# Sharath-girish/Shacira

Hardware: AMD Instinct MI355X
Metric: hash-grid samples/sec fwd+bwd (16 lvl, F=2) (higher is better)
Workload: dtype f32

## Files before the change

shacira_amd/csrc/bwd_bin_front.h:

```cpp
#pragma once

#include "bwd_bin_types.h"

namespace shacira {

template <typename T, int F, bool GMAX>
__global__ __launch_bounds__(256) void transpose_grad_kernel(const T *__restrict__ go, float *__restrict__ gT,
                                                             int64_t N, int64_t NP, int L, int lb, int le,
                                                             uint32_t *__restrict__ gmax) {
    __shared__ uint32_t s_max[SHACIRA_MAX_LODS];
    if (GMAX && threadIdx.x < SHACIRA_MAX_LODS) s_max[threadIdx.x] = 0;
    struct alignas(sizeof(T) * F) PieceIn { T v[F]; };
    struct alignas(sizeof(float) * F) PieceOut { float v[F]; };
    extern __shared__ __align__(16) unsigned char s_raw_g[];
    PieceOut *s_tile = reinterpret_cast<PieceOut *>(s_raw_g);
    const int pitch = L + 1;
    const int64_t s0 = (int64_t)blockIdx.x * 256;
    const int ns = (int)((N - s0 < 256) ? (N - s0) : 256);
    const PieceIn *in = reinterpret_cast<const PieceIn *>(go) + s0 * L;
    const int total = ns * L;
    for (int e = threadIdx.x; e < total; e += 256) {
        const int sm = e / L, l = e - sm * L;
        const PieceIn p = in[e];
        PieceOut q;
// ... 173 lines not shown
            v += r512;
            if (v >= VPR) { v -= VPR; ++sm; }
        }
        for (int e = (int)threadIdx.x + kFrontThreads * UL; e < total; e += kFrontThreads) {
            park1(__builtin_nontemporal_load(src_of(e, sm, v)), sm, v);
            sm += q512;
            v += r512;
            if (v >= VPR) { v -= VPR; ++sm; }
        }
        lds_barrier();
        if constexpr (COUNT) {
            uint32_t *row = cnt + (size_t)(tile0 + r) * plan.total_buckets;
            const bool close = plan.pad > 1u && ((uint32_t)((tile0 + r + 1) % (int64_t)cps) == 0u || tile0 + r + 1 == tiles);
#pragma unroll
            for (int j = 0; j < HE; ++j) {
                const int hc = hcol_of(j);
                if (hc >= 0) {
                    const uint32_t h = s_hist[threadIdx.x + j * kFrontThreads];
                    s_hist[threadIdx.x + j * kFrontThreads] = 0;
                    row[hc] = h;
                    hacc[j] += h;
                    hsum[j] += h;
                    if (close) {
                        hsum[j] += (0u - hacc[j]) & (plan.pad - 1u);
                        hacc[j] = 0;
                    }
                }
            }
        }
        const int work = (le - lb) << nvec_log2;
        for (int idx = threadIdx.x; idx < work; idx += kFrontThreads) {
            const int l = lb + (idx >> nvec_log2), smo = (idx & ((1 << nvec_log2) - 1)) << M_LOG2;
            uint32_t m = 0;
            if (smo < ns) {
                const f32x4 val = *reinterpret_cast<const f32x4 *>(&s_tile[l * pitch + smo]);
                float *dst = gT + ((int64_t)l * NP + s0 + smo) * F;
                if (smo + M <= ns) {
                    if constexpr (sizeof(T) == 4) *reinterpret_cast<f32x4 *>(dst) = val;
                    else __builtin_nontemporal_store(val, reinterpret_cast<f32x4 *>(dst));
                    if constexpr (GMAX) {
#pragma unroll
                        for (int j = 0; j < 4; ++j) {
                            const uint32_t b = __float_as_uint(fabsf(val[j]));
                            m = b > m ? b : m;
                        }
                    }
                } else {
#pragma unroll
                    for (int j = 0; j < F; ++j) {
                        dst[j] = val[j];
                        if constexpr (GMAX) {
                            const uint32_t b = __float_as_uint(fabsf(val[j]));
                            m = b > m ? b : m;
                        }
                    }
                }
            }
            if constexpr (GMAX) {
#pragma unroll
                for (int off = 32; off > 0; off >>= 1) {
                    const uint32_t o = __shfl_xor(m, off, 64);
                    m = o > m ? o : m;
                }
                if ((threadIdx.x & 63) == 0 && m) atomicMax(&s_max[l], m);
            }
        }
        lds_barrier();
    }
    __syncthreads();
    if constexpr (COUNT) {
        uint32_t *mine = totals + (size_t)(blockIdx.x % kTotalShards) * kMaxBuckets;
#pragma unroll
        for (int j = 0; j < HE; ++j) {
            const int hc = hcol_of(j);
            if (hc >= 0 && hsum[j]) atomicAdd(&mine[hc], hsum[j]);
        }
    }
    if constexpr (GMAX) {
        if ((int)threadIdx.x >= lb && (int)threadIdx.x < le && s_max[threadIdx.x])
            atomicMax(&gmax[threadIdx.x], s_max[threadIdx.x]);
    }
}

__global__ __launch_bounds__(1024) void bin_scan_buckets_kernel(const uint32_t *__restrict__ totals,
                                                                uint64_t *__restrict__ base,
                                                                uint32_t *__restrict__ unit_first,
                                                                UnitDesc *__restrict__ unit_desc, uint32_t nb,
                                                                BinPlan plan,
                                                                uint32_t *__restrict__ work_counter,
                                                                unsigned long long *__restrict__ cursor,
                                                                const uint32_t *__restrict__ gmax) {
    __shared__ uint64_t s_items[kMaxBuckets + 2];
    __shared__ uint32_t s_units[kMaxBuckets + 2];
    __shared__ uint64_t s_wave_items[16];
    __shared__ uint32_t s_wave_units[16];
    const uint32_t t = threadIdx.x, lane = t & 63, wave = t >> 6;
    if (t == 0) work_counter[0] = 0;
    uint64_t c[2];
    uint32_t u[2], lv_of[2], ck[2];
#pragma unroll
    for (int k = 0; k < 2; ++k) {
        const uint32_t b = 2 * t + k;
        c[k] = 0u;
        if (b < nb)
            for (int sh = 0; sh < kTotalShards; ++sh) c[k] += totals[(size_t)sh * kMaxBuckets + b];
        uint32_t lvl = plan.blevel[0];
#pragma unroll
        for (uint32_t q = 1; q < SHACIRA_MAX_LODS; ++q)
            if (q < plan.nbl && plan.bstart[q] <= b) lvl = plan.blevel[q];
        lv_of[k] = lvl;
        ck[k] = plan.chunk;
        u[k] = (c[k] >> 32) ? (uint32_t)((c[k] + ck[k] - 1) / ck[k]) : (c[k] ? ((uint32_t)c[k] - 1u) / ck[k] + 1u : 0u);
    }
    uint64_t ci = c[0] + c[1];
    uint32_t ui = u[0] + u[1];
#pragma unroll
    for (int off = 1; off < 64; off <<= 1) {
        const uint64_t nc = __shfl_up(ci, off, 64);
        const uint32_t nu = __shfl_up(ui, off, 64);
        if (lane >= (uint32_t)off) { ci += nc; ui += nu; }
    }
    if (lane == 63) { s_wave_items[wave] = ci; s_wave_units[wave] = ui; }
    __syncthreads();
    uint64_t wc = 0;
    uint32_t wu = 0;
    for (uint32_t w = 0; w < wave; ++w) { wc += s_wave_items[w]; wu += s_wave_units[w]; }
    const uint64_t ex_items = wc + ci - (c[0] + c[1]);
    const uint32_t ex_units = wu + ui - (u[0] + u[1]);
    s_items[2 * t] = ex_items;
    s_items[2 * t + 1] = ex_items + c[0];
    s_units[2 * t] = ex_units;
    s_units[2 * t + 1] = ex_units + u[0];
    if (t == 1023) {
        s_items[kMaxBuckets] = ex_items + c[0] + c[1];
        s_units[kMaxBuckets] = ex_units + u[0] + u[1];
    }
    __syncthreads();
    for (uint32_t b = t; b <= nb; b += 1024) {
        base[b] = s_items[b];
        cursor[b] = s_items[b];
        unit_first[b] = s_units[b];
    }
#pragma unroll
    for (int k = 0; k < 2; ++k) {
        const uint32_t b = 2 * t + k;
        if (b < nb) {
            const uint32_t lvl = lv_of[k];
            const uint32_t gm = (gmax != nullptr && u[k] > 0) ? gmax[lvl] : 0u;
            for (uint32_t q = 0; q < u[k]; ++q) {
                UnitDesc d;
                d.begin = s_items[b] + (uint64_t)q * ck[k];
                const uint64_t bucket_end = s_items[b] + c[k];
                d.end = (d.begin + ck[k] < bucket_end) ? (d.begin + ck[k]) : bucket_end;
                d.bucket = b;
                d.level = lvl;
                d.single = u[k] == 1 ? 1u : 0u;
                d.gmax_bits = gm;
                unit_desc[s_units[b] + q] = d;
            }
        }
    }
}

template <int DIM>
__global__ __launch_bounds__(kBinThreads) void bin_count_levels_kernel(LevelTable lt, BinPlan plan,
                                                                       const float *__restrict__ coords,
                                                                       uint32_t *__restrict__ totals,
                                                                       uint32_t *__restrict__ cnt, int64_t sample0,
                                                                       int64_t N) {
    __shared__ uint32_t s_hist[SHACIRA_MAX_LODS][kMaxLevelBuckets];
    constexpr int kTileD = TileOf<DIM>::value;
    constexpr int SPT = kTileD / kBinThreads;
    const uint32_t tile = blockIdx.x;
    for (uint32_t e = threadIdx.x; e < plan.nbl * kMaxLevelBuckets; e += kBinThreads) (&s_hist[0][0])[e] = 0;
    double t[SPT][DIM];
    bool live[SPT];
#pragma unroll
    for (int u = 0; u < SPT; ++u) {
        const int64_t i = sample0 + (int64_t)tile * kTileD + threadIdx.x + u * kBinThreads;
        live[u] = i < N;
        load_unit_coords<DIM>(coords, i, N, t[u]);
    }
    __syncthreads();
#pragma unroll 1
    for (uint32_t bi = blockIdx.y; bi < plan.nbl; bi += gridDim.y) {
        const uint32_t lvl = plan.blevel[bi];
        const BinLevel bl = plan.lv[lvl];
        const int32_t res = lt.res[lvl];
        const float hi = lt.hi[lvl];
        const bool dense = lt.dense[lvl] != 0;
#pragma unroll
        for (int u = 0; u < SPT; ++u) {
            if (!live[u]) continue;
            if (bl.compact) {
                if constexpr (DIM == 3) {
                    atomicAdd(&s_hist[bi][axis_pos(t[u][2], res, hi) / bl.slab], 2u);
                } else {
                    atomicAdd(&s_hist[bi][compact2d_line(axis_pos(t[u][1], res, hi), (uint32_t)res) / bl.slab], 1u);
                }
                continue;
            }
            uint32_t bk[1 << (DIM - 1)];
            bool ok[1 << (DIM - 1)];
            enumerate_buckets<DIM>(t[u], res, hi, dense, lt.mask, bl, bk, ok);
#pragma unroll
            for (int q = 0; q < (1 << (DIM - 1)); ++q)
                if (ok[q]) atomicAdd(&s_hist[bi][bk[q]], 1u);
        }
    }
    __syncthreads();
    for (uint32_t bi = blockIdx.y; bi < plan.nbl; bi += gridDim.y) {
        const BinLevel bl = plan.lv[plan.blevel[bi]];
        for (uint32_t b = threadIdx.x; b < bl.nb; b += kBinThreads)
        {
            const uint32_t c = (s_hist[bi][b] + plan.pad - 1u) & ~(plan.pad - 1u);
            cnt[(size_t)tile * plan.total_buckets + bl.bucket0 + b] = s_hist[bi][b];
            if (c)
                atomicAdd(&totals[(size_t)((blockIdx.x + blockIdx.y) % kTotalShards) * kMaxBuckets + bl.bucket0 + b], c);
        }
    }
}

__global__ __launch_bounds__(256) void zero_unowned_rows_kernel(float *__restrict__ acc,
                                                                const int32_t *__restrict__ first_idx, LevelTable lt,
                                                                BinPlan plan, uint32_t *__restrict__ words,
                                                                uint32_t nwords) {
    if ((int)blockIdx.y == lt.num_lods) {
        for (uint32_t i = blockIdx.x * 256 + threadIdx.x; i < nwords; i += gridDim.x * 256) words[i] = 0u;
        return;
    }
    const int l = blockIdx.y, F = lt.feature_dim;
// ... 35 lines not shown
```

shacira_amd/csrc/bwd_bin_passes.h:

```cpp
#pragma once

#include "bwd_bin_types.h"

namespace shacira {

#ifdef SHACIRA_SCATTER_WAVES
#define SHACIRA_SCATTER_ATTR __attribute__((amdgpu_waves_per_eu(SHACIRA_SCATTER_WAVES)))
#else
#define SHACIRA_SCATTER_ATTR
#endif
template <int DIM, int F, int FMT, bool STREAM = true>
__global__ __launch_bounds__((ScatterThreads<DIM, F, FMT>::value)) SHACIRA_SCATTER_ATTR void bin_scatter_kernel(LevelTable lt, BinPlan plan,
                                                                  const float *__restrict__ coords,
                                                                  const float *__restrict__ gT,
                                                                  unsigned long long *__restrict__ cursor,
                                                                  const uint32_t *__restrict__ cnt, uint32_t cps,
                                                                  uint32_t cnt_rows,
                                                                  typename ItemSel<F, FMT>::type *__restrict__ items,
                                                                  int64_t sample0, int64_t N, int64_t gpitch,
                                                                  float *__restrict__ zero_acc,
                                                                  const int32_t *__restrict__ first_idx,
                                                                  const uint32_t *__restrict__ unit_first,
                                                                  int cstride = DIM) {
    typedef typename ItemSel<F, FMT>::type ItemT;
    constexpr bool H = FMT == 1;
    constexpr bool P12 = FMT == 2;
    static_assert(!P12 || (DIM == 3 && F == 2), "12-byte units: 3-D, F = 2");
    constexpr int NP = 1 << (DIM - 1);
    constexpr int kTileD = TileOf<DIM>::value;
    constexpr int kThreads = ScatterThreads<DIM, F, FMT>::value;
    constexpr int SPT = kTileD / kThreads;
    constexpr int kScatterSplit = ScatterSplit<ItemT>::value;
    constexpr int kStage = kTileD * NP / kScatterSplit;
    static_assert(kStage % 2 == 0, "two-slot items never straddle a window");
    extern __shared__ __align__(16) unsigned char s_raw[];
    ItemT *s_items = reinterpret_cast<ItemT *>(s_raw);
    uint8_t *s_bucket = reinterpret_cast<uint8_t *>(s_items + (kScatterSplit == 1 ? plan.stage_cap : (uint32_t)kStage));
    __shared__ uint32_t s_hist[kMaxLevelBuckets];
    __shared__ uint32_t s_start[kMaxLevelBuckets + 1];
    __shared__ uint64_t s_gbase[kMaxLevelBuckets];

#ifdef SCATTER_LEVEL_FAST
    const uint32_t tile = blockIdx.y, bi = blockIdx.x;
#else
    const uint32_t tile = blockIdx.x, bi = blockIdx.y;
#endif
    const uint32_t lvl = plan.blevel[bi];
    const BinLevel bl = plan.lv[lvl];
    if (threadIdx.x < kMaxLevelBuckets) s_hist[threadIdx.x] = 0;
    __syncthreads();
    const int32_t res = lt.res[lvl];
    const float hi = lt.hi[lvl];
    const bool dense = lt.dense[lvl] != 0;

    PairSlot ps[SPT][NP];
    uint32_t rank[SPT][NP];
    float fx[SPT];
    float g[SPT][F];
    float fyz[SPT][2];
    const bool compact = bl.compact != 0;
    constexpr uint32_t kCompactSlots = (DIM == 3) ? 2u : 1u;
    float craw[SPT][DIM], graw[SPT][F];
#pragma unroll
    for (int u = 0; u < SPT; ++u) {
        int64_t i = sample0 + (int64_t)tile * kTileD + threadIdx.x + u * kThreads;
        i = i < N ? i : N - 1;
#ifdef ABL_NO_LOAD
        i = (i * 2654435761ll) & 1023;
#endif
#pragma unroll
        for (int a = 0; a < DIM; ++a) craw[u][a] = coords[i * cstride + a];
        const float *gp = gT + ((int64_t)lvl * gpitch + i) * F;
        if constexpr (F == 2) {
            const float2 v = *reinterpret_cast<const float2 *>(gp);
            graw[u][0] = v.x; graw[u][1] = v.y;
        } else {
#pragma unroll
            for (int j = 0; j < F; ++j) graw[u][j] = gp[j];
        }
    }
    const bool reserver = threadIdx.x >= 64 && threadIdx.x - 64 < bl.nb;
    unsigned long long run_base = 0ull;
    if (reserver) {
        const uint32_t gb = bl.bucket0 + threadIdx.x - 64;
        const uint32_t *row = cnt + (size_t)tile * cps * plan.total_buckets + gb;
        uint32_t c = 0;
        for (uint32_t k = 0; k < cps && tile * cps + k < cnt_rows; ++k) c += row[(size_t)k * plan.total_buckets];
        c = (c + plan.pad - 1u) & ~(plan.pad - 1u);
#ifdef ABL_NO_CURSOR
        if (c) run_base = cursor[gb] + (unsigned long long)tile * c;
#else
        if (c) run_base = atomicAdd(&cursor[gb], (unsigned long long)c);
#endif
    }
#pragma unroll
    for (int u = 0; u < SPT; ++u) {
        const int k = threadIdx.x + u * kThreads;
        const int64_t i = sample0 + (int64_t)tile * kTileD + k;
        const bool live = i < N;
        double t[DIM];
#pragma unroll
        for (int a = 0; a < DIM; ++a) t[a] = axis_unit(craw[u][a]);
#pragma unroll
        for (int j = 0; j < F; ++j) g[u][j] = graw[u][j];
        if (compact) {
            if constexpr (DIM == 3) {
                int32_t pp[3];
                float ff[3], gg[3];
#pragma unroll
                for (int a = 0; a < 3; ++a) axis_transform(t[a], res, hi, pp[a], ff[a], gg[a]);
                const uint32_t r = (uint32_t)res, b = (uint32_t)pp[2] / bl.slab;
                const uint32_t local = ((uint32_t)pp[2] - b * bl.slab) * r * r + (uint32_t)pp[1] * r + (uint32_t)pp[0];
                fx[u] = ff[0];
                fyz[u][0] = ff[1];
                fyz[u][1] = ff[2];
#pragma unroll
                for (int q = 0; q < NP; ++q) {
                    ps[u][q].bucket = b;
                    ps[u][q].key = 0;
                    ps[u][q].wrest = 0.0f;
                }
                ps[u][0].key = local | (1u << 26);
            } else {
                int32_t pp[2];
                float ff[2], gg[2];
#pragma unroll
                for (int a = 0; a < 2; ++a) axis_transform(t[a], res, hi, pp[a], ff[a], gg[a]);
                const uint32_t r = (uint32_t)res, b = compact2d_line((uint32_t)pp[1], r) / bl.slab;
                const uint32_t local = ((uint32_t)pp[1] - b * bl.slab) * r + (uint32_t)pp[0];
                fx[u] = ff[0];
                fyz[u][0] = ff[1];
                fyz[u][1] = 0.0f;
                ps[u][0].bucket = b;
                ps[u][0].key = local | (1u << 26);
                ps[u][0].wrest = 0.0f;
                ps[u][1].bucket = b;
                ps[u][1].key = 0;
                ps[u][1].wrest = 0.0f;
            }
        } else {
            enumerate_pairs<DIM>(t, res, hi, dense, lt.mask, bl, plan.BR, fx[u], ps[u]);
        }
#pragma unroll
        for (int q = 0; q < NP; ++q) {
            if (!live) ps[u][q].key = 0;
            rank[u][q] = (ps[u][q].key >> 26) ? atomicAdd(&s_hist[ps[u][q].bucket], compact ? kCompactSlots : 1u) : 0u;
        }
    }
    lds_barrier();
    if (threadIdx.x < 64) {
        const uint32_t lane = threadIdx.x;
        const uint32_t pm = plan.pad - 1u;
        const uint32_t c0 = (2 * lane < bl.nb) ? ((s_hist[2 * lane] + pm) & ~pm) : 0u;
        const uint32_t c1 = (2 * lane + 1 < bl.nb) ? ((s_hist[2 * lane + 1] + pm) & ~pm) : 0u;
        uint32_t incl = c0 + c1;
#pragma unroll
        for (int off = 1; off < 64; off <<= 1) {
            const uint32_t nbr = __shfl_up(incl, off, 64);
            if (lane >= (uint32_t)off) incl += nbr;
        }
        const uint32_t excl = incl - (c0 + c1);
        if (2 * lane < bl.nb) s_start[2 * lane] = excl;
        if (2 * lane + 1 < bl.nb) s_start[2 * lane + 1] = excl + c0;
        if (lane == 63) s_start[bl.nb] = incl;
    }
    lds_barrier();
    if (kScatterSplit == 1 && plan.pad > 1u && threadIdx.x < bl.nb) {
        const uint32_t b = threadIdx.x;
        for (uint32_t pos = s_start[b] + s_hist[b]; pos < s_start[b + 1]; ++pos) {
            uint32_t *w = reinterpret_cast<uint32_t *>(&s_items[pos]);
#pragma unroll
            for (int k = 0; k < (int)(sizeof(ItemT) / 4); ++k) w[k] = 0u;
            s_bucket[pos] = (uint8_t)b;
        }
    }
    const uint32_t staged = s_start[bl.nb];
// ... 49 lines not shown
                    } else {
                        s_items[pos] = pack_item12(ps[u][q].key, fx[u], dense, g[u][0] * ps[u][q].wrest, g[u][1] * ps[u][q].wrest);
                        s_bucket[pos] = (uint8_t)ps[u][q].bucket;
                    }
                    continue;
                }
                if constexpr (H && F == 2) {
                    if (compact) {
                        ItemHC c;
                        c.key = ps[u][q].key;
                        c.fx = (uint16_t)(fx[u] * 65536.0f);
                        c.fy = (uint16_t)(fyz[u][0] * 65536.0f);
                        c.fz = (uint16_t)(fyz[u][1] * 65536.0f);
                        c.pad = 0;
                        c.g = __floats2half2_rn(g[u][0], g[u][1]);
                        *reinterpret_cast<ItemHC *>(&s_items[pos]) = c;
                        s_bucket[pos] = (uint8_t)ps[u][q].bucket;
                        s_bucket[pos + 1] = (uint8_t)ps[u][q].bucket;
                    } else {
                        ItemH it;
                        it.key = pack_half_key(ps[u][q].key, fx[u], dense);
                        it.a = __floats2half2_rn(g[u][0] * ps[u][q].wrest, g[u][1] * ps[u][q].wrest);
                        s_items[pos] = it;
                        s_bucket[pos] = (uint8_t)ps[u][q].bucket;
                    }
                    continue;
                }
                if constexpr (!H && !P12) {
                Item<F> it;
                it.key = ps[u][q].key;
                it.fx = fx[u];
                if constexpr (DIM == 2 && !H) {
                    if (compact) {
                        uint32_t w0, w1;
                        pack_compact2d(ps[u][q].key, fx[u], fyz[u][0], w0, w1);
                        it.key = w0;
                        it.fx = __uint_as_float(w1);
#pragma unroll
                        for (int j = 0; j < F; ++j) it.a[j] = g[u][j];
                        *reinterpret_cast<Item<F> *>(&s_items[pos]) = it;
                        s_bucket[pos] = (uint8_t)ps[u][q].bucket;
                        continue;
                    }
                }
                if (compact) {
                    if constexpr (F == 2) {
                        it.a[0] = fyz[u][0];
                        it.a[1] = fyz[u][1];
                        *reinterpret_cast<Item<F> *>(&s_items[pos]) = it;
                        Item<F> it2;
                        it2.key = 0;
                        it2.fx = g[u][0];
                        it2.a[0] = g[u][1];
                        it2.a[1] = 0.0f;
                        *reinterpret_cast<Item<F> *>(&s_items[pos + 1]) = it2;
                        s_bucket[pos] = (uint8_t)ps[u][q].bucket;
                        s_bucket[pos + 1] = (uint8_t)ps[u][q].bucket;
                    } else if constexpr (F == 4) {
                        it.a[0] = fyz[u][0];
                        it.a[1] = fyz[u][1];
                        it.a[2] = g[u][0];
                        it.a[3] = g[u][1];
                        *reinterpret_cast<Item<F> *>(&s_items[pos]) = it;
                        Item<F> it2;
                        it2.key = 0;
                        it2.fx = g[u][2];
                        it2.a[0] = g[u][3];
                        it2.a[1] = 0.0f; it2.a[2] = 0.0f; it2.a[3] = 0.0f;
                        *reinterpret_cast<Item<F> *>(&s_items[pos + 1]) = it2;
                        s_bucket[pos] = (uint8_t)ps[u][q].bucket;
                        s_bucket[pos + 1] = (uint8_t)ps[u][q].bucket;
                    }
                } else {
#pragma unroll
                    for (int j = 0; j < F; ++j) it.a[j] = g[u][j] * ps[u][q].wrest;
                    *reinterpret_cast<Item<F> *>(&s_items[pos]) = it;
                    s_bucket[pos] = (uint8_t)ps[u][q].bucket;
                }
                }
            }
        }
    }
    if (wi == 0) {
        if (reserver) s_gbase[threadIdx.x - 64] = run_base;
        __syncthreads();
    } else {
        lds_barrier();
    }
    const uint32_t in_window = (kScatterSplit == 1 || staged - w0 < (uint32_t)kStage) ? (staged - w0) : (uint32_t)kStage;
#ifndef ABL_NO_STORE
    for (uint32_t pos = threadIdx.x; pos < in_window; pos += kThreads) {
        const uint32_t b = s_bucket[pos];
        store_item_nt<STREAM>(items + s_gbase[b] + (w0 + pos - s_start[b]), s_items[pos]);
    }
#endif
    if (kScatterSplit > 1 && wi + 1u < n_win) lds_barrier();
    }
    if (zero_acc != nullptr && !dense) {
        for (uint32_t b = tile; b < bl.nb; b += plan.num_tiles) {
            const uint32_t gb = bl.bucket0 + b;
            if (unit_first[gb + 1] - unit_first[gb] == 1u) continue;
            const uint32_t row0 = b * bl.rows_pb;
            const uint32_t nrows = (bl.used - row0 < bl.rows_pb) ? (bl.used - row0) : bl.rows_pb;
            float *dst = zero_acc + ((int64_t)first_idx[lvl] + row0) * F;
            for (uint32_t e = threadIdx.x; e < nrows * (uint32_t)F; e += kThreads) dst[e] = 0.0f;
        }
    }
}

#ifdef CONSUME_TRACE
__device__ unsigned long long g_consume_trace[16384 * 8];
__device__ unsigned int g_consume_trace_n;
#define CTRACE(k) do { if (threadIdx.x == 0) ctr[k] = wall_clock64(); } while (0)
#else
#define CTRACE(k) do { } while (0)
#endif
template <int F, bool FX, int FMT, class Hook>
__device__ __forceinline__ void consume_unit(const LevelTable &lt, const BinPlan &plan, const int32_t *__restrict__ first_idx,
                                             const UnitDesc d, const typename ItemSel<F, FMT>::type *__restrict__ items,
                                             float *__restrict__ grad_table, int force_atomic, int headroom, double *s_acc,
                                             Hook &&hook, __half *__restrict__ half_out = nullptr) {
    constexpr bool H = FMT == 1;
    constexpr bool P12 = FMT == 2;
    const uint32_t gb = (uint32_t)__builtin_amdgcn_readfirstlane((int)d.bucket);
    const uint32_t lvl = (uint32_t)__builtin_amdgcn_readfirstlane((int)d.level);
    const BinLevel bl = plan.lv[lvl];
    const uint32_t b = gb - bl.bucket0;
    const uint32_t r1 = (uint32_t)lt.res[lvl];
    const bool two_d = plan.pairs == 2u;
    const uint32_t row0 = bl.compact ? b * bl.slab * (two_d ? r1 : r1 * r1) : b * bl.rows_pb;
    const uint32_t nrows = (bl.used - row0 < bl.rows_pb) ? (bl.used - row0) : bl.rows_pb;

    FxScale fx{1.0, 1.0, false};
    if constexpr (FX) fx = fx_scale_of(d.gmax_bits, headroom);
    unsigned long long *s_fix = reinterpret_cast<unsigned long long *>(s_acc);
#ifdef CONSUME_TRACE
    unsigned long long ctr[8] = {0, 0, 0, 0, 0, 0, 0, 0};
    struct TraceOut {
        unsigned long long *c; UnitDesc dd;
        __device__ ~TraceOut() {
            if (threadIdx.x == 0) {
                c[5] = wall_clock64();
                const unsigned int slot = atomicAdd(&g_consume_trace_n, 1u);
                if (slot < 16384u) {
                    unsigned long long *o = g_consume_trace + (size_t)slot * 8;
                    o[0] = ((unsigned long long)dd.level << 32) | dd.bucket;
                    o[1] = dd.end - dd.begin;
                    for (int k = 0; k < 6; ++k) o[2 + k] = c[k];
                }
            }
        }
    } trace_out{ctr, d};
#endif
    CTRACE(0);
    auto zero_image = [&]() {
        for (uint32_t e = threadIdx.x; e < nrows * F; e += kConsumeThreads) s_acc[e] = 0.0;
        lds_barrier();
    };
    const uint64_t begin = d.begin, end = d.end;
    auto stream = [&](uint64_t first, uint64_t lim, uint64_t stride, auto &&load, auto &&proc) {
        uint64_t p0 = first;
        load(p0);
        CTRACE(1);
        zero_image();
        CTRACE(2);
        proc();
        CTRACE(3);
// ... 663 lines not shown
```

shacira_amd/csrc/hashgrid_bwd_bin.hip:

```cpp
#include <mutex>

#include <cstring>

#include "bwd_bin_types.h"
#include "bwd_bin_front.h"
#include "bwd_bin_passes.h"
#include "bwd_brick.h"
#include <hip/hip_ext.h>

namespace shacira {

static inline size_t align_up(size_t v, size_t a) { return (v + a - 1) / a * a; }

static void make_plan(int dim, int dtype, const LevelTable &lt, int64_t n_batch, BinPlan &plan, int acc_kib,
                      bool one_image_compact, uint32_t skip_mask = 0u, int64_t n_call = 0);
static inline bool half_items(int dtype, const LevelTable &lt);
static inline int item_format(int dim, int dtype, const LevelTable &lt, int64_t n);
static inline size_t item_unit_bytes(int fmt, const LevelTable &lt);
#ifndef SHACIRA_RUN_ALIGN
#define SHACIRA_RUN_ALIGN 64
#endif
#ifndef SHACIRA_PAD_HALF
#define SHACIRA_PAD_HALF 0
#endif
// ... 214 lines not shown
        plan.bnb[q] = q < plan.nbl ? plan.lv[plan.blevel[q]].nb : 0u;
    }
    plan.total_buckets = nbk;
    plan.BR = BR;
    plan.num_tiles = (uint32_t)((n_batch + tile_samples(dim) - 1) / tile_samples(dim));
    plan.pairs = 1u << (dim - 1);
    uint64_t chunk = (uint64_t)n_batch * plan.pairs / 48 + 1024;
    if (chunk < 8192) chunk = 8192;
    if (chunk > (1u << 22)) chunk = 1u << 22;
    plan.pad = 1;
    {
        const int fmt_p = item_format(dim, dtype, lt, n_call);
        const size_t unit = item_unit_bytes(fmt_p, lt);
        const uint32_t tile_units = (uint32_t)tile_samples(dim) * plan.pairs;
        uint32_t maxnb = 0;
        for (uint32_t q = 0; q < plan.nbl; ++q) maxnb = plan.lv[plan.blevel[q]].nb > maxnb ? plan.lv[plan.blevel[q]].nb : maxnb;
        bool windows = false;
#ifdef SHACIRA_SCATTER_SPLIT
        windows = SHACIRA_SCATTER_SPLIT > 1;
#endif
        if (opt().bwd_run_pad != 0 && !windows && plan.nbl > 0 && n_call >= SHACIRA_FX_MIN &&
            ((fmt_p != 1 && (unit == 16 || unit == 12)) || (SHACIRA_PAD_HALF && fmt_p == 1 && (unit == 8 || unit == 16)))) {
            const uint32_t P = unit == 12 ? (uint32_t)(SHACIRA_RUN_ALIGN / 4) : (uint32_t)(SHACIRA_RUN_ALIGN / unit);
            const size_t staged = (size_t)(tile_units + maxnb * (P - 1u)) * (unit + 1);
            if (staged <= (size_t)78 * 1024 || (size_t)tile_units * (unit + 1) > (size_t)78 * 1024) plan.pad = P;
        }
        plan.stage_cap = tile_units + maxnb * (plan.pad - 1u);
    }
    const uint32_t cmask = plan.pad > 2u ? plan.pad - 1u : 1u;
    plan.chunk = (uint32_t)chunk & ~cmask;
    for (uint32_t q = 0; q < plan.nbl; ++q) {
        BinLevel &bl = plan.lv[plan.blevel[q]];
        bl.chunk = plan.chunk;
        CountLevel &c = plan.cl[q];
        c.res = lt.res[plan.blevel[q]];
        c.hi = lt.hi[plan.blevel[q]];
        c.shift = bl.shift;
        c.m_lo = (uint32_t)bl.magicG;
        c.m_hi = (uint32_t)(bl.magicG >> 32);
        c.kind = lt.dense[plan.blevel[q]] ? 2u : 0u;
        if (bl.compact) {
            const uint32_t m = ((1u << 18) + bl.slab - 1u) / bl.slab;
            bool exact = m < (1u << 18) || bl.slab == 1;
            for (uint32_t pz = 0; pz < (uint32_t)c.res && exact; ++pz) exact = ((pz * m) >> 18) == pz / bl.slab;
            c.kind = 1u;
            c.m_lo = exact ? m : 0u;
            c.m_hi = bl.slab;
        }
    }
    plan.chunk_min = plan.chunk;
}

static inline bool half_items(int dtype, const LevelTable &lt) {
    return dtype == SHACIRA_F16 && (lt.feature_dim == 2 || lt.feature_dim == 4);
}
static inline int item_format(int dim, int dtype, const LevelTable &lt, int64_t n) {
    if (half_items(dtype, lt)) return 1;
    if (dim == 3 && lt.feature_dim == 2 && dtype == SHACIRA_F32 && n >= SHACIRA_FX_MIN && opt().bwd_item12 == 1) return 2;
    return 0;
}
static inline size_t item_unit_bytes(int fmt, const LevelTable &lt) {
    if (fmt == 1) return lt.feature_dim == 2 ? 8 : 16;
    if (fmt == 2) return 12;
    return 8 + 4 * (size_t)lt.feature_dim;
}

static int64_t bin_batch_samples(int dim, int dtype, const LevelTable &lt, int64_t n) {
    const size_t item = item_unit_bytes(item_format(dim, dtype, lt, n), lt);
    BinPlan plan;
    make_plan(dim, dtype, lt, kTile, plan, choose_acc_kib(dim, dtype, lt, n), one_image_compact_rule(n));
    const size_t per_sample = (size_t)(plan.nbl ? plan.nbl : 1) * (1u << (dim - 1)) * item;
    int64_t cap = (int64_t)(((size_t)opt().bin_batch_mib << 20) / per_sample);
    cap = cap / tile_samples(dim) * tile_samples(dim);
    if (cap < tile_samples(dim)) cap = tile_samples(dim);
    return n < cap ? n : cap;
}

struct BinWorkspace {
    float *gT;
    unsigned char *items;
    uint32_t *totals;
    uint32_t *gmax;
    uint64_t *base;
    unsigned long long *cursor;
    uint32_t *cnt;
    uint32_t *unit_first;
    UnitDesc *unit_desc;
    uint32_t *work_counter;
    float *acc32;
    size_t bytes;
};

static inline int64_t level_pitch(int64_t n) { return (n + 1) & ~(int64_t)1; }

static bool table_all_direct(int dim, int dtype, const LevelTable &lt, int64_t n) {
    LevelTable full = lt;
    full.level_begin = 0;
    full.level_end = lt.num_lods;
    BinPlan plan;
    make_plan(dim, dtype, full, kTile, plan, choose_acc_kib(dim, dtype, full, n), one_image_compact_rule(n));
    return plan.nbl == 0;
}

static uint64_t slots_per_sample(const BinPlan &plan) {
    uint64_t slots = 0;
    for (uint32_t q = 0; q < plan.nbl; ++q) {
        const BinLevel &bl = plan.lv[plan.blevel[q]];
        slots += bl.compact ? (plan.pairs == 4u ? 2u : 1u) : plan.pairs;
    }
    return slots;
}

static int front_tile(int L, int F, uint32_t nbl, int64_t n, size_t *shmem);

static void brick_levels_of_call(int dim, int dtype, const LevelTable &lt, int64_t n, const SortedBatch *sb, bool zero_table,
                                 bool grad_aligned, BrickPlan &brick, uint32_t &skip_mask) {
    brick.nlev = 0;
    skip_mask = 0u;
    if (dim != 3 || sb == nullptr) return;
    const int L = lt.num_lods, F = lt.feature_dim;
    const bool multi = bin_batch_samples(dim, dtype, lt, n) < n;
    const int kvec0 = (int)(16 / ((dtype == SHACIRA_F32 ? 4 : 2) * F));
    const int bopt = opt().bwd_brick;
    const bool wanted = bopt == 1 || (bopt < 0 && F == 2 && dtype == SHACIRA_F32);
    if (!wanted || multi || lt.stage_flags != 0 || !zero_table || n < SHACIRA_FX_MIN || n * L >= ((int64_t)1 << 31) ||
        table_all_direct(dim, dtype, lt, n) || (L % kvec0) != 0 || !grad_aligned)
        return;
    if (!make_brick_plan(lt, n, *sb, opt().bwd_brick_lo, opt().bwd_brick_hi, opt().bwd_brick_span,
                         (size_t)(opt().bwd_brick_fork == 2 ? 30 : 64) * 1024, brick)) {
        brick.nlev = 0;
        return;
    }
    for (uint32_t q = 0; q < brick.nlev; ++q) skip_mask |= 1u << brick.lv[q].level;
    BinPlan rest;
    make_plan(dim, dtype, lt, n, rest, choose_acc_kib(dim, dtype, lt, n), one_image_compact_rule(n), skip_mask, n);
    size_t sh0 = 0;
    if (rest.nbl == 0 || front_tile(L, F, rest.nbl, n, &sh0) <= 0) {
        skip_mask = 0u;
        brick.nlev = 0;
    }
}

static BinWorkspace carve(int dim, int dtype, const LevelTable &lt, int64_t n, void *ws, uint32_t skip_mask = 0u) {
    BinPlan plan;
    const int64_t nb = bin_batch_samples(dim, dtype, lt, n);
    make_plan(dim, dtype, lt, nb, plan, choose_acc_kib(dim, dtype, lt, n), one_image_compact_rule(n), skip_mask, n);
    const size_t item = item_unit_bytes(item_format(dim, dtype, lt, n), lt);
    size_t off = 0;
    auto take = [&](size_t bytes) { size_t o = off; off = align_up(off + bytes, 256); return o; };
    const bool no_stage = table_all_direct(dim, dtype, lt, n);
    const size_t o_gT = take(no_stage ? 0 : (size_t)level_pitch(n) * lt.num_lods * lt.feature_dim * sizeof(float));
    const size_t o_ctrl = take((size_t)(kTotalShards * kMaxBuckets + SHACIRA_MAX_LODS) * sizeof(uint32_t));
    const uint64_t pad_units = (uint64_t)plan.num_tiles * plan.total_buckets * (plan.pad - 1u);
    const size_t o_items = take(((size_t)nb * slots_per_sample(plan) + (size_t)pad_units) * item);
    const size_t o_base = take((size_t)(kMaxBuckets + 2) * sizeof(uint64_t));
    const size_t o_cur = take((size_t)(kMaxBuckets + 2) * sizeof(uint64_t));
    const size_t o_cnt = take((size_t)(nb / 128 + 8) * plan.total_buckets * sizeof(uint32_t));
    const size_t o_unit = take((size_t)(kMaxBuckets + 2) * sizeof(uint32_t));
    const uint64_t max_items_ws = (uint64_t)nb * plan.nbl * plan.pairs + pad_units;
    const size_t o_ub = take((size_t)(max_items_ws / plan.chunk_min + plan.total_buckets + 2) * sizeof(UnitDesc));
    const size_t o_wc = take(256);
    const size_t o_acc = take(dtype == SHACIRA_F16 ? (size_t)lt.table_rows * lt.feature_dim * sizeof(float) : 0);
    BinWorkspace w{};
    unsigned char *p = static_cast<unsigned char *>(ws);
    if (p) {
        w.gT = reinterpret_cast<float *>(p + o_gT);
        w.items = p + o_items;
        w.totals = reinterpret_cast<uint32_t *>(p + o_ctrl);
        w.gmax = w.totals + (size_t)kTotalShards * kMaxBuckets;
        w.base = reinterpret_cast<uint64_t *>(p + o_base);
        w.cursor = reinterpret_cast<unsigned long long *>(p + o_cur);
        w.cnt = reinterpret_cast<uint32_t *>(p + o_cnt);
        w.unit_first = reinterpret_cast<uint32_t *>(p + o_unit);
        w.unit_desc = reinterpret_cast<UnitDesc *>(p + o_ub);
        w.work_counter = reinterpret_cast<uint32_t *>(p + o_wc);
        w.acc32 = reinterpret_cast<float *>(p + o_acc);
    }
    w.bytes = off;
    return w;
}

static void resolve_call(int dim, int dtype, const LevelTable &lt, int64_t n, const SortedBatch *sb, bool zero_table,
                         bool grad_aligned, BrickPlan &brick, uint32_t &skip_mask) {
    const bool auto12 = opt().bwd_item12 < 0;
    if (auto12) {
        const bool brick_shape = sb != nullptr && dim == 3 && lt.feature_dim == 2 && dtype == SHACIRA_F32 &&
                                 lt.level_begin == 0 && lt.level_end == lt.num_lods && lt.stage_flags == 0 && zero_table &&
                                 opt().bwd_brick != 0;
        options_resolve_item12(brick_shape ? 1 : 0);
    }
    brick_levels_of_call(dim, dtype, lt, n, sb, zero_table, grad_aligned, brick, skip_mask);
    if (auto12 && brick.nlev == 0) options_resolve_item12(0);
}
static inline uint32_t carve_skip(int dtype, uint32_t skip_mask) { return dtype == SHACIRA_F32 ? skip_mask : 0u; }

size_t bin_workspace_bytes(int dim, int dtype, const LevelTable &lt, int64_t n) {
    return carve(dim, dtype, lt, n, nullptr).bytes;
}

size_t bin_workspace_bytes_planned(int dim, int dtype, const LevelTable &lt, int64_t n, bool whole, bool grad_aligned) {
    SortedBatch sb{};
    sample_plan_grid(dim, n, sb);
    BrickPlan brick;
    uint32_t skip_mask = 0;
    resolve_call(dim, dtype, lt, n, &sb, whole, grad_aligned, brick, skip_mask);
    return carve(dim, dtype, lt, n, nullptr, carve_skip(dtype, skip_mask)).bytes;
}

float *bin_acc32(int dim, int dtype, const LevelTable &lt, int64_t n, void *workspace) {
    return carve(dim, dtype, lt, n, workspace).acc32;
}

#define SHACIRA_CHECK_LAUNCH()                 \
    do {                                       \
        hipError_t e_ = hipGetLastError();     \
        if (e_ != hipSuccess) return e_;       \
    } while (0)
#define SHACIRA_CHECK(expr)                    \
    do {                                       \
        hipError_t e_ = (expr);                \
        if (e_ != hipSuccess) return e_;       \
    } while (0)

struct SideStream {
    hipStream_t stream = nullptr;
    hipEvent_t fork = nullptr, join = nullptr, staged = nullptr;
    hipEvent_t bfork = nullptr, bjoin = nullptr;
};
static hipError_t side_stream(SideStream **out) {
    static thread_local SideStream per_device[kMaxDevices];
    int dev = 0;
    SHACIRA_CHECK(hipGetDevice(&dev));
    if (dev < 0 || dev >= kMaxDevices) return hipErrorInvalidDevice;
    SideStream &ss = per_device[dev];
    if (!ss.stream) {
        hipStream_t st;
        hipEvent_t a, b, c, d, e;
        SHACIRA_CHECK(hipStreamCreateWithFlags(&st, hipStreamNonBlocking));
        SHACIRA_CHECK(hipEventCreateWithFlags(&a, hipEventDisableTiming));
        SHACIRA_CHECK(hipEventCreateWithFlags(&b, hipEventDisableTiming));
        SHACIRA_CHECK(hipEventCreateWithFlags(&c, hipEventDisableTiming));
        SHACIRA_CHECK(hipEventCreateWithFlags(&d, hipEventDisableTiming));
        SHACIRA_CHECK(hipEventCreateWithFlags(&e, hipEventDisableTiming));
        ss.fork = a;
        ss.join = b;
        ss.staged = c;
        ss.bfork = d;
        ss.bjoin = e;
        ss.stream = st;
    }
    *out = &ss;
    return hipSuccess;
}

// ... 141 lines not shown
                else if (front_counts) SHACIRA_FRONT(__half, false, true);
                else SHACIRA_FRONT(__half, false, false);
            }
#undef SHACIRA_FRONT
#undef SHACIRA_FRONT_SORTED
        } else {
            const uint32_t blocks = (uint32_t)((n + 255) / 256);
            const size_t shmem = (size_t)256 * (L + 1) * F * sizeof(float);
            if (dtype == SHACIRA_F32 && use_fx)
                hipLaunchKernelGGL((transpose_grad_kernel<float, F, true>), dim3(blocks), dim3(256), shmem, s,
                                   static_cast<const float *>(grad_out), w.gT, n, NP, L, t_lb, t_le, w.gmax);
            else if (dtype == SHACIRA_F32)
                hipLaunchKernelGGL((transpose_grad_kernel<float, F, false>), dim3(blocks), dim3(256), shmem, s,
                                   static_cast<const float *>(grad_out), w.gT, n, NP, L, t_lb, t_le, nullptr);
            else if (use_fx)
                hipLaunchKernelGGL((transpose_grad_kernel<__half, F, true>), dim3(blocks), dim3(256), shmem, s,
                                   static_cast<const __half *>(grad_out), w.gT, n, NP, L, t_lb, t_le, w.gmax);
            else
                hipLaunchKernelGGL((transpose_grad_kernel<__half, F, false>), dim3(blocks), dim3(256), shmem, s,
                                   static_cast<const __half *>(grad_out), w.gT, n, NP, L, t_lb, t_le, nullptr);
        }
        SHACIRA_CHECK_LAUNCH();
    }
    if (fork) {
        SHACIRA_CHECK(hipEventRecord(ss->staged, s));
        SHACIRA_CHECK(hipStreamWaitEvent(ss->stream, ss->staged, 0));
    }
    if (brick_mode == 1) SHACIRA_CHECK(fork_brick());
    if (whole.ngroups > 0) {
        const BinPlan &plan = whole;
        uint32_t bpg = (plan.ngroups > 1 ? 256u : 512u) / plan.ngroups;
        const uint32_t need = (uint32_t)((n + 2047) / 2048);
        if (bpg > need) bpg = need;
        if (bpg < 1) bpg = 1;
        const size_t acc_bytes = (size_t)plan.BR * F * sizeof(double);
        const dim3 grid(bpg, plan.ngroups);
        const int headroom = fx_headroom(((uint64_t)n / bpg + kConsumeThreads) * (1u << DIM));
        const uint32_t *gm = (need_T && use_fx) ? w.gmax : nullptr;
        if (need_T)
            hipLaunchKernelGGL((direct_accumulate_kernel<DIM, F, float, true, true>), grid, dim3(kConsumeThreads),
                               acc_bytes, zs, lt, plan, first_idx, cptr, w.gT, acc, n, NP, gm, headroom, cstride);
        else if (dtype == SHACIRA_F32)
            hipLaunchKernelGGL((direct_accumulate_kernel<DIM, F, float, false, true>), grid, dim3(kConsumeThreads),
                               acc_bytes, zs, lt, plan, first_idx, coords, static_cast<const float *>(grad_out), acc, n,
                               NP, gm, headroom);
        else
            hipLaunchKernelGGL((direct_accumulate_kernel<DIM, F, __half, false, true>), grid, dim3(kConsumeThreads),
                               acc_bytes, zs, lt, plan, first_idx, coords, static_cast<const __half *>(grad_out), acc, n,
                               NP, gm, headroom);
        SHACIRA_CHECK_LAUNCH();
    }
    if (fork) SHACIRA_CHECK(hipEventRecord(ss->join, ss->stream));
    if (whole.nbl == 0) return hipSuccess;
    constexpr int NPAIR = 1 << (DIM - 1);
    const int fmt = item_format(DIM, dtype, lt, n);
    const bool half = fmt == 1;
    auto stage_bytes = [&](const BinPlan &pl) -> size_t {
        const size_t isz = fmt == 2 ? sizeof(Item12) : half ? sizeof(typename ItemSel<F, true>::type) : sizeof(Item<F>);
        const int split = half ? ScatterSplit<typename ItemSel<F, true>::type>::value : ScatterSplit<Item<F>>::value;
        const size_t units = split == 1 ? (size_t)pl.stage_cap : (size_t)TileOf<DIM>::value * NPAIR / split;
        return units * (isz + 1);
    };
#ifdef SCATTER_LEVEL_FAST
#define SCATTER_GRID(pl) dim3((pl).nbl, (pl).num_tiles)
#else
#define SCATTER_GRID(pl) dim3((pl).num_tiles, (pl).nbl)
#endif
    bool first_batch = true;
    for (int64_t s0 = 0; s0 < n; s0 += nb) {
        const int64_t hi = (s0 + nb < n) ? (s0 + nb) : n;
        BinPlan plan;
        make_plan(DIM, dtype, lt, hi - s0, plan, acc_kib, oic, skip_mask, n);
        if (!first_batch) {
            hipLaunchKernelGGL(zero_words_kernel, dim3(32), dim3(256), 0, s, w.totals, (uint32_t)kTotalShards * kMaxBuckets);
            SHACIRA_CHECK_LAUNCH();
        }
        const bool fused_now = front_counts && first_batch;
        if (!fused_now) {
            hipLaunchKernelGGL((bin_count_levels_kernel<DIM>), count_grid(plan), dim3(kBinThreads), 0, s, lt, plan, coords,
                               w.totals, w.cnt, s0, hi);
            SHACIRA_CHECK_LAUNCH();
        }
        first_batch = false;
        hipLaunchKernelGGL(bin_scan_buckets_kernel, dim3(1), dim3(1024), 0, s, w.totals, w.base, w.unit_first, w.unit_desc,
                           plan.total_buckets, plan, w.work_counter, w.cursor, use_fx ? w.gmax : nullptr);
        SHACIRA_CHECK_LAUNCH();
        float *zacc = selective ? acc : nullptr;
        const uint32_t cps = fused_now ? (uint32_t)(TileOf<DIM>::value / ts16) : 1u;
        const uint32_t cnt_rows = fused_now ? (uint32_t)((n + ts16 - 1) / ts16) : plan.num_tiles;
        bool fork_signalled = false;
        if (fmt == 2) {
            if constexpr (DIM == 3 && F == 2) {
                hipStreamCaptureStatus cap = hipStreamCaptureStatusNone;
                if (brick_mode == 2 && opt().bwd_ext_fork != 0 && hipStreamIsCapturing(s, &cap) == hipSuccess &&
                    cap == hipStreamCaptureStatusNone) {
                    hipExtLaunchKernelGGL((bin_scatter_kernel<DIM, F, 2>), SCATTER_GRID(plan),
                                          dim3(ScatterThreads<DIM, F, 2>::value), (uint32_t)stage_bytes(plan), s, nullptr,
                                          bss->bfork, 0u, lt, plan, cptr, (const float *)w.gT, w.cursor, (const uint32_t *)w.cnt, cps, cnt_rows,
                                          reinterpret_cast<Item12 *>(w.items), s0, hi, NP, zacc, first_idx,
                                          (const uint32_t *)w.unit_first, cstride);
                    fork_signalled = true;
                } else {
                    hipLaunchKernelGGL((bin_scatter_kernel<DIM, F, 2>), SCATTER_GRID(plan), dim3(ScatterThreads<DIM, F, 2>::value),
                                       stage_bytes(plan), s, lt, plan, cptr, w.gT, w.cursor, w.cnt, cps, cnt_rows,
                                       reinterpret_cast<Item12 *>(w.items), s0, hi, NP, zacc, first_idx, w.unit_first, cstride);
                }
            }
        } else if (half)
            hipLaunchKernelGGL((bin_scatter_kernel<DIM, F, true>), SCATTER_GRID(plan), dim3(ScatterThreads<DIM, F, 1>::value),
                               stage_bytes(plan), s, lt, plan, cptr, w.gT, w.cursor, w.cnt, cps, cnt_rows,
                               reinterpret_cast<typename ItemSel<F, true>::type *>(w.items), s0, hi, NP, zacc, first_idx,
                               w.unit_first, cstride);
        else if (use_fx)
            hipLaunchKernelGGL((bin_scatter_kernel<DIM, F, false>), SCATTER_GRID(plan), dim3(ScatterThreads<DIM, F, 0>::value),
                               stage_bytes(plan), s, lt, plan, cptr, w.gT, w.cursor, w.cnt, cps, cnt_rows,
                               reinterpret_cast<Item<F> *>(w.items), s0, hi, NP, zacc, first_idx, w.unit_first, cstride);
        else
            hipLaunchKernelGGL((bin_scatter_kernel<DIM, F, false, false>), SCATTER_GRID(plan), dim3(ScatterThreads<DIM, F, 0>::value),
                               stage_bytes(plan), s, lt, plan, cptr, w.gT, w.cursor, w.cnt, cps, cnt_rows,
                               reinterpret_cast<Item<F> *>(w.items), s0, hi, NP, zacc, first_idx, w.unit_first, cstride);
        SHACIRA_CHECK_LAUNCH();
        if (fork) SHACIRA_CHECK(hipStreamWaitEvent(s, ss->join, 0));
        if (brick_mode == 2) {
            if (fork_signalled) {
                SHACIRA_CHECK(hipStreamWaitEvent(bss->stream, bss->bfork, 0));
                SHACIRA_CHECK(launch_brick(bss->stream, bss->bjoin));
            } else {
                SHACIRA_CHECK(fork_brick());
            }
        }
        const uint64_t max_items = (uint64_t)(hi - s0) * plan.nbl * NPAIR +
                                   (uint64_t)plan.num_tiles * plan.total_buckets * (plan.pad - 1u);
        uint32_t grid_units = (uint32_t)(max_items / plan.chunk_min) + plan.total_buckets + 1;
        const size_t acc_bytes = (size_t)plan.BR * F * sizeof(double);
        uint32_t *wc = (opt().bwd_persistent != 0 && n >= SHACIRA_PERSIST_MIN) ? w.work_counter : nullptr;
        if (wc != nullptr && grid_units > 512u) grid_units = 512u;
        const int headroom = use_fx ? fx_headroom((uint64_t)plan.chunk + 1) : -1;
        const int fa = multi ? 1 : 0;
        __half *hout = direct_half ? half_table : nullptr;
        if (fmt == 2) {
            if constexpr (DIM == 3 && F == 2)
                hipLaunchKernelGGL((bin_consume_kernel<F, true, 2>), dim3(grid_units), dim3(kConsumeThreads), acc_bytes, s, lt,
                                   plan, first_idx, w.unit_first, w.unit_desc, reinterpret_cast<const Item12 *>(w.items), acc,
                                   fa, headroom, wc);
        } else if (half && use_fx)
            hipLaunchKernelGGL((bin_consume_kernel<F, true, true>), dim3(grid_units), dim3(kConsumeThreads), acc_bytes, s,
                               lt, plan, first_idx, w.unit_first, w.unit_desc,
                               reinterpret_cast<const typename ItemSel<F, true>::type *>(w.items), acc, fa, headroom, wc, hout);
        else if (half)
            hipLaunchKernelGGL((bin_consume_kernel<F, false, true>), dim3(grid_units), dim3(kConsumeThreads), acc_bytes, s,
                               lt, plan, first_idx, w.unit_first, w.unit_desc,
                               reinterpret_cast<const typename ItemSel<F, true>::type *>(w.items), acc, fa, headroom, wc, hout);
        else if (use_fx)
            hipLaunchKernelGGL((bin_consume_kernel<F, true, false>), dim3(grid_units), dim3(kConsumeThreads), acc_bytes, s, lt,
                               plan, first_idx, w.unit_first, w.unit_desc,
                               reinterpret_cast<const Item<F> *>(w.items), acc, fa, headroom, wc);
        else if (!half)
            hipLaunchKernelGGL((bin_consume_kernel<F, false, false>), dim3(grid_units), dim3(kConsumeThreads), acc_bytes, s, lt,
                               plan, first_idx, w.unit_first, w.unit_desc,
                               reinterpret_cast<const Item<F> *>(w.items), acc, fa, headroom, wc);
        SHACIRA_CHECK_LAUNCH();
    }
    if (brick_mode == 0) SHACIRA_CHECK(launch_brick(s));
    if (brick_mode > 0) SHACIRA_CHECK(hipStreamWaitEvent(s, bss->bjoin, 0));
    if (direct_half) {
        hipLaunchKernelGGL(f32_to_f16_skip_kernel, dim3(128, (uint32_t)L), dim3(256), 0, s, acc, half_table, first_idx, lt,
                           whole, w.unit_first, F);
        SHACIRA_CHECK_LAUNCH();
        if (converted != nullptr) *converted = true;
    }
    return hipSuccess;
}

template <class ItemT> static constexpr size_t stage_max(size_t tile_units) {
    constexpr size_t split = ScatterSplit<ItemT>::value;
    constexpr size_t padu = split != 1 ? 0 : sizeof(ItemT) == 16 ? SHACIRA_RUN_ALIGN / 16 - 1 : sizeof(ItemT) == 12 ? SHACIRA_RUN_ALIGN / 4 - 1
                            : (SHACIRA_PAD_HALF && sizeof(ItemT) == 8) ? SHACIRA_RUN_ALIGN / 8 - 1 : 0;
    return (tile_units / split + (size_t)kMaxLevelBuckets * padu) * (sizeof(ItemT) + 1);
}

hipError_t bin_backward(int dim, int dtype, const LevelTable &lt, const int32_t *first_idx, const float *coords,
                        const void *grad_out, float *acc, void *workspace, int64_t n, hipStream_t s, bool zero_table,
                        void *half_table, bool *converted, const SortedBatch *sb) {
    if (converted != nullptr) *converted = false;
    __half *ht = (dtype == SHACIRA_F16) ? static_cast<__half *>(half_table) : nullptr;
    BrickPlan brick;
    uint32_t skip_mask = 0;
    resolve_call(dim, dtype, lt, n, sb, zero_table, (reinterpret_cast<uintptr_t>(grad_out) & 15u) == 0, brick, skip_mask);
    const BinWorkspace w = carve(dim, dtype, lt, n, workspace, carve_skip(dtype, skip_mask));
    static PerDeviceOnce once;
    const hipError_t attr_err = once.run([]() -> hipError_t {
        hipError_t attr_err = hipSuccess;
        auto set = [&attr_err](const void *fn, size_t bytes) {
            if (bytes <= 64 * 1024 || bytes > 160 * 1024) return;
            hipError_t e = hipFuncSetAttribute(fn, hipFuncAttributeMaxDynamicSharedMemorySize, (int)bytes);
            if (e != hipSuccess) attr_err = e;
        };
#define SHACIRA_T_ATTR(TT, FF)                                                                           \
        set(reinterpret_cast<const void *>(&transpose_grad_kernel<TT, FF, true>), 140 * 1024);          \
        set(reinterpret_cast<const void *>(&transpose_grad_kernel<TT, FF, false>), 140 * 1024);         \
        set(reinterpret_cast<const void *>(&front16_kernel<2, TT, FF, true, true>), 156 * 1024);        \
        set(reinterpret_cast<const void *>(&front16_kernel<2, TT, FF, true, false>), 156 * 1024);       \
// ... 66 lines not shown
```

Baseline: 1.415 billion.

## Replace per-tile atomic cursor reservation with deterministic prefix-scanned run offsets

```diff
diff --git a/shacira_amd/csrc/bwd_bin_front.h b/shacira_amd/csrc/bwd_bin_front.h
--- a/shacira_amd/csrc/bwd_bin_front.h
+++ b/shacira_amd/csrc/bwd_bin_front.h
@@ -279,14 +279,82 @@
     }
 }
 
-__global__ __launch_bounds__(1024) void bin_scan_buckets_kernel(const uint32_t *__restrict__ totals,
-                                                                uint64_t *__restrict__ base,
-                                                                uint32_t *__restrict__ unit_first,
-                                                                UnitDesc *__restrict__ unit_desc, uint32_t nb,
-                                                                BinPlan plan,
-                                                                uint32_t *__restrict__ work_counter,
-                                                                unsigned long long *__restrict__ cursor,
-                                                                const uint32_t *__restrict__ gmax) {
+constexpr int kScanThreads = 1024;
+constexpr int kScanCols = 16;
+constexpr int kScanChunks = kScanThreads / kScanCols;
+constexpr int kScanRows = 32;
+static_assert(kScanChunks == 64, "one wave scans one column's chunk sums");
+__device__ __forceinline__ void scan_run_offsets(uint32_t *__restrict__ cnt, uint32_t group, uint32_t nb, uint32_t pad,
+                                                 uint32_t cps, uint32_t cnt_rows) {
+    __shared__ uint32_t s_chunk[kScanCols][kScanChunks + 1];
+    const uint32_t col = threadIdx.x % kScanCols, chunk = threadIdx.x / kScanCols;
+    const uint32_t lane = threadIdx.x & 63, wave = threadIdx.x >> 6;
+    const uint32_t gb = group * kScanCols + col;
+    const bool live = gb < nb;
+    uint32_t *colp = cnt + (live ? gb : nb - 1u);
+    const uint32_t pm = pad - 1u;
+    uint32_t carry = 0;
+    for (uint32_t row0 = 0; row0 < cnt_rows; row0 += (uint32_t)(kScanChunks * kScanRows)) {
+        const uint32_t r0 = row0 + chunk * (uint32_t)kScanRows;
+        const uint32_t left = r0 < cnt_rows ? cnt_rows - r0 : 0u;
+        const uint32_t nvalid = left < (uint32_t)kScanRows ? left : (uint32_t)kScanRows;
+        const uint32_t *p = colp + (size_t)(nvalid ? r0 : cnt_rows - 1u) * nb;
+        uint32_t v[kScanRows];
+#pragma unroll
+        for (int k = 0; k < kScanRows; ++k) {
+            v[k] = *p;
+            p += ((uint32_t)k + 1u < nvalid) ? nb : 0u;
+        }
+        uint32_t run = 0, acc = 0;
+#pragma unroll
+        for (int k = 0; k < kScanRows; ++k) {
+            const uint32_t h = ((uint32_t)k < nvalid) ? v[k] : 0u;
+            v[k] = run;
+            acc += h;
+            if ((((uint32_t)k + 1u) & (cps - 1u)) == 0u) {
+                run += (acc + pm) & ~pm;
+                acc = 0;
+            }
+        }
+        s_chunk[col][chunk] = run;
+        __syncthreads();
+        {
+            const uint32_t t = s_chunk[wave][lane];
+            uint32_t incl = t;
+#pragma unroll
+            for (int off = 1; off < 64; off <<= 1) {
+                const uint32_t nbr = __shfl_up(incl, off, 64);
+                if (lane >= (uint32_t)off) incl += nbr;
+            }
+            s_chunk[wave][lane] = incl - t;
+            if (lane == 63) s_chunk[wave][kScanChunks] = incl;
+        }
+        __syncthreads();
+        const uint32_t off0 = carry + s_chunk[col][chunk];
+        carry += s_chunk[col][kScanChunks];
+        uint32_t *w = colp + (size_t)r0 * nb;
+#pragma unroll
+        for (int k = 0; k < kScanRows; ++k) {
+            if (((uint32_t)k & (cps - 1u)) == 0u && (uint32_t)k < nvalid && live) *w = off0 + v[k];
+            w += nb;
+        }
+        __syncthreads();
+    }
+}
+
+__global__ __launch_bounds__(kScanThreads) void bin_scan_buckets_kernel(const uint32_t *__restrict__ totals,
+                                                                        uint64_t *__restrict__ base,
+                                                                        uint32_t *__restrict__ unit_first,
+                                                                        UnitDesc *__restrict__ unit_desc, uint32_t nb,
+                                                                        BinPlan plan,
+                                                                        uint32_t *__restrict__ work_counter,
+                                                                        const uint32_t *__restrict__ gmax,
+                                                                        uint32_t *__restrict__ cnt, uint32_t cps,
+                                                                        uint32_t cnt_rows) {
+    if (blockIdx.x != 0) {
+        scan_run_offsets(cnt, blockIdx.x - 1u, nb, plan.pad, cps, cnt_rows);
+        return;
+    }
     __shared__ uint64_t s_items[kMaxBuckets + 2];
     __shared__ uint32_t s_units[kMaxBuckets + 2];
     __shared__ uint64_t s_wave_items[16];
@@ -294,7 +362,7 @@
     const uint32_t t = threadIdx.x, lane = t & 63, wave = t >> 6;
     if (t == 0) work_counter[0] = 0;
     uint64_t c[2];
-    uint32_t u[2], lv_of[2], ck[2];
+    uint32_t u[2], lv_of[2], ck[2], gm_of[2];
 #pragma unroll
     for (int k = 0; k < 2; ++k) {
         const uint32_t b = 2 * t + k;
@@ -306,6 +374,7 @@
         for (uint32_t q = 1; q < SHACIRA_MAX_LODS; ++q)
             if (q < plan.nbl && plan.bstart[q] <= b) lvl = plan.blevel[q];
         lv_of[k] = lvl;
+        gm_of[k] = gmax != nullptr ? gmax[lvl] : 0u;
         ck[k] = plan.chunk;
         u[k] = (c[k] >> 32) ? (uint32_t)((c[k] + ck[k] - 1) / ck[k]) : (c[k] ? ((uint32_t)c[k] - 1u) / ck[k] + 1u : 0u);
     }
@@ -335,7 +404,6 @@
     __syncthreads();
     for (uint32_t b = t; b <= nb; b += 1024) {
         base[b] = s_items[b];
-        cursor[b] = s_items[b];
         unit_first[b] = s_units[b];
     }
 #pragma unroll
@@ -343,7 +411,7 @@
         const uint32_t b = 2 * t + k;
         if (b < nb) {
             const uint32_t lvl = lv_of[k];
-            const uint32_t gm = (gmax != nullptr && u[k] > 0) ? gmax[lvl] : 0u;
+            const uint32_t gm = gm_of[k];
             for (uint32_t q = 0; q < u[k]; ++q) {
                 UnitDesc d;
                 d.begin = s_items[b] + (uint64_t)q * ck[k];
diff --git a/shacira_amd/csrc/bwd_bin_passes.h b/shacira_amd/csrc/bwd_bin_passes.h
--- a/shacira_amd/csrc/bwd_bin_passes.h
+++ b/shacira_amd/csrc/bwd_bin_passes.h
@@ -13,9 +13,8 @@
 __global__ __launch_bounds__((ScatterThreads<DIM, F, FMT>::value)) SHACIRA_SCATTER_ATTR void bin_scatter_kernel(LevelTable lt, BinPlan plan,
                                                                   const float *__restrict__ coords,
                                                                   const float *__restrict__ gT,
-                                                                  unsigned long long *__restrict__ cursor,
-                                                                  const uint32_t *__restrict__ cnt, uint32_t cps,
-                                                                  uint32_t cnt_rows,
+                                                                  const uint64_t *__restrict__ base,
+                                                                  const uint32_t *__restrict__ run_off, uint32_t cps,
                                                                   typename ItemSel<F, FMT>::type *__restrict__ items,
                                                                   int64_t sample0, int64_t N, int64_t gpitch,
                                                                   float *__restrict__ zero_acc,
@@ -79,19 +78,11 @@
             for (int j = 0; j < F; ++j) graw[u][j] = gp[j];
         }
     }
-    const bool reserver = threadIdx.x >= 64 && threadIdx.x - 64 < bl.nb;
-    unsigned long long run_base = 0ull;
-    if (reserver) {
+    const bool placer = threadIdx.x >= 64 && threadIdx.x - 64 < bl.nb;
+    uint64_t run_base = 0ull;
+    if (placer) {
         const uint32_t gb = bl.bucket0 + threadIdx.x - 64;
-        const uint32_t *row = cnt + (size_t)tile * cps * plan.total_buckets + gb;
-        uint32_t c = 0;
-        for (uint32_t k = 0; k < cps && tile * cps + k < cnt_rows; ++k) c += row[(size_t)k * plan.total_buckets];
-        c = (c + plan.pad - 1u) & ~(plan.pad - 1u);
-#ifdef ABL_NO_CURSOR
-        if (c) run_base = cursor[gb] + (unsigned long long)tile * c;
-#else
-        if (c) run_base = atomicAdd(&cursor[gb], (unsigned long long)c);
-#endif
+        run_base = base[gb] + run_off[(size_t)tile * cps * plan.total_buckets + gb];
     }
 #pragma unroll
     for (int u = 0; u < SPT; ++u) {
@@ -307,7 +298,7 @@
         }
     }
     if (wi == 0) {
-        if (reserver) s_gbase[threadIdx.x - 64] = run_base;
+        if (placer) s_gbase[threadIdx.x - 64] = run_base;
         __syncthreads();
     } else {
         lds_barrier();
diff --git a/shacira_amd/csrc/hashgrid_bwd_bin.hip b/shacira_amd/csrc/hashgrid_bwd_bin.hip
--- a/shacira_amd/csrc/hashgrid_bwd_bin.hip
+++ b/shacira_amd/csrc/hashgrid_bwd_bin.hip
@@ -320,7 +320,6 @@
     uint32_t *totals;
     uint32_t *gmax;
     uint64_t *base;
-    unsigned long long *cursor;
     uint32_t *cnt;
     uint32_t *unit_first;
     UnitDesc *unit_desc;
@@ -392,7 +391,6 @@
     const uint64_t pad_units = (uint64_t)plan.num_tiles * plan.total_buckets * (plan.pad - 1u);
     const size_t o_items = take(((size_t)nb * slots_per_sample(plan) + (size_t)pad_units) * item);
     const size_t o_base = take((size_t)(kMaxBuckets + 2) * sizeof(uint64_t));
-    const size_t o_cur = take((size_t)(kMaxBuckets + 2) * sizeof(uint64_t));
     const size_t o_cnt = take((size_t)(nb / 128 + 8) * plan.total_buckets * sizeof(uint32_t));
     const size_t o_unit = take((size_t)(kMaxBuckets + 2) * sizeof(uint32_t));
     const uint64_t max_items_ws = (uint64_t)nb * plan.nbl * plan.pairs + pad_units;
@@ -407,7 +405,6 @@
         w.totals = reinterpret_cast<uint32_t *>(p + o_ctrl);
         w.gmax = w.totals + (size_t)kTotalShards * kMaxBuckets;
         w.base = reinterpret_cast<uint64_t *>(p + o_base);
-        w.cursor = reinterpret_cast<unsigned long long *>(p + o_cur);
         w.cnt = reinterpret_cast<uint32_t *>(p + o_cnt);
         w.unit_first = reinterpret_cast<uint32_t *>(p + o_unit);
         w.unit_desc = reinterpret_cast<UnitDesc *>(p + o_ub);
@@ -715,12 +712,14 @@
             SHACIRA_CHECK_LAUNCH();
         }
         first_batch = false;
-        hipLaunchKernelGGL(bin_scan_buckets_kernel, dim3(1), dim3(1024), 0, s, w.totals, w.base, w.unit_first, w.unit_desc,
-                           plan.total_buckets, plan, w.work_counter, w.cursor, use_fx ? w.gmax : nullptr);
+        const uint32_t cps = fused_now ? (uint32_t)(TileOf<DIM>::value / ts16) : 1u;
+        const uint32_t cnt_rows = fused_now ? (uint32_t)((n + ts16 - 1) / ts16) : plan.num_tiles;
+        static_assert(TileOf<DIM>::value / 128 <= kScanRows, "a thread of the bucket scan walks whole scatter tiles");
+        hipLaunchKernelGGL(bin_scan_buckets_kernel, dim3(1u + (plan.total_buckets + kScanCols - 1u) / kScanCols),
+                           dim3(kScanThreads), 0, s, w.totals, w.base, w.unit_first, w.unit_desc, plan.total_buckets, plan,
+                           w.work_counter, use_fx ? w.gmax : nullptr, w.cnt, cps, cnt_rows);
         SHACIRA_CHECK_LAUNCH();
         float *zacc = selective ? acc : nullptr;
-        const uint32_t cps = fused_now ? (uint32_t)(TileOf<DIM>::value / ts16) : 1u;
-        const uint32_t cnt_rows = fused_now ? (uint32_t)((n + ts16 - 1) / ts16) : plan.num_tiles;
         bool fork_signalled = false;
         if (fmt == 2) {
             if constexpr (DIM == 3 && F == 2) {
@@ -729,28 +728,28 @@
                     cap == hipStreamCaptureStatusNone) {
                     hipExtLaunchKernelGGL((bin_scatter_kernel<DIM, F, 2>), SCATTER_GRID(plan),
                                           dim3(ScatterThreads<DIM, F, 2>::value), (uint32_t)stage_bytes(plan), s, nullptr,
-                                          bss->bfork, 0u, lt, plan, cptr, (const float *)w.gT, w.cursor, (const uint32_t *)w.cnt, cps, cnt_rows,
+                                          bss->bfork, 0u, lt, plan, cptr, (const float *)w.gT, (const uint64_t *)w.base, (const uint32_t *)w.cnt, cps,
                                           reinterpret_cast<Item12 *>(w.items), s0, hi, NP, zacc, first_idx,
                                           (const uint32_t *)w.unit_first, cstride);
                     fork_signalled = true;
                 } else {
                     hipLaunchKernelGGL((bin_scatter_kernel<DIM, F, 2>), SCATTER_GRID(plan), dim3(ScatterThreads<DIM, F, 2>::value),
-                                       stage_bytes(plan), s, lt, plan, cptr, w.gT, w.cursor, w.cnt, cps, cnt_rows,
+                                       stage_bytes(plan), s, lt, plan, cptr, w.gT, w.base, w.cnt, cps,
                                        reinterpret_cast<Item12 *>(w.items), s0, hi, NP, zacc, first_idx, w.unit_first, cstride);
                 }
             }
         } else if (half)
             hipLaunchKernelGGL((bin_scatter_kernel<DIM, F, true>), SCATTER_GRID(plan), dim3(ScatterThreads<DIM, F, 1>::value),
-                               stage_bytes(plan), s, lt, plan, cptr, w.gT, w.cursor, w.cnt, cps, cnt_rows,
+                               stage_bytes(plan), s, lt, plan, cptr, w.gT, w.base, w.cnt, cps,
                                reinterpret_cast<typename ItemSel<F, true>::type *>(w.items), s0, hi, NP, zacc, first_idx,
                                w.unit_first, cstride);
         else if (use_fx)
             hipLaunchKernelGGL((bin_scatter_kernel<DIM, F, false>), SCATTER_GRID(plan), dim3(ScatterThreads<DIM, F, 0>::value),
-                               stage_bytes(plan), s, lt, plan, cptr, w.gT, w.cursor, w.cnt, cps, cnt_rows,
+                               stage_bytes(plan), s, lt, plan, cptr, w.gT, w.base, w.cnt, cps,
                                reinterpret_cast<Item<F> *>(w.items), s0, hi, NP, zacc, first_idx, w.unit_first, cstride);
         else
             hipLaunchKernelGGL((bin_scatter_kernel<DIM, F, false, false>), SCATTER_GRID(plan), dim3(ScatterThreads<DIM, F, 0>::value),
-                               stage_bytes(plan), s, lt, plan, cptr, w.gT, w.cursor, w.cnt, cps, cnt_rows,
+                               stage_bytes(plan), s, lt, plan, cptr, w.gT, w.base, w.cnt, cps,
                                reinterpret_cast<Item<F> *>(w.items), s0, hi, NP, zacc, first_idx, w.unit_first, cstride);
         SHACIRA_CHECK_LAUNCH();
         if (fork) SHACIRA_CHECK(hipStreamWaitEvent(s, ss->join, 0));
```

Result: faster. 1.472 billion (median of 6 runs) (+4.0%).
